# paTRICK-swk/D3DP

Hardware: AMD Instinct MI355X
Metric: pose-hypotheses/sec (H x clips) at F=243, J=17, H=20, K=10 (higher is better)
Workload: dtype f16x2-split operands on fp16 MFMA, f32 accumulate (fp32-class: meets 1e-3 mm)

## Files before the change

d3dp_amd/csrc/attention_x2.hip:

```cpp
#include "common.h"
#include "kernels.h"
#include "ta_common.h"
#include "attn_frag.h"

#ifndef D3DP_ATTN_OVERLAP
#define D3DP_ATTN_OVERLAP 0
#endif
#ifndef D3DP_ATTN_KPIPE
#define D3DP_ATTN_KPIPE 0
#endif
#ifndef D3DP_ATTN_MIXLO
#define D3DP_ATTN_MIXLO 0
#endif
#ifndef D3DP_ATTN_W16
#define D3DP_ATTN_W16 0
#endif
#ifndef D3DP_ATTN_STAMP
#define D3DP_ATTN_STAMP 0
#endif

namespace {

__device__ __forceinline__ f16x8 as_f16x8(bf16x8 v) { return __builtin_bit_cast(f16x8, v); }

// ... 732 lines not shown
          ph[e] = hh;
          pl[e] = (f16)fmaf(y, 1.0f, -(float)hh);
        }
        psum += __shfl_xor(psum, 16, 64);
        psum += __shfl_xor(psum, 32, 64);
        lrun = fmaf(lrun, alpha, psum);
#pragma unroll
        for (int dn = 0; dn < ND; ++dn) o[dn] *= alpha;
        if constexpr (HD == 64) {
          ta_tr_chunk<PLANE>(fv, t >> 1, ph, pl, o);
        } else {
          FragBasesT<HD> fc = fb;
#pragma unroll
          for (int dn = 0; dn < ND; ++dn) fc.v[dn] += (t >> 1) * 32 * H::ROWB;
          pv_chunk_x2_seq<0>(fc, PLANE, ph, pl, o);
        }
      }
    }
    if (active && q < n)
      store_o_x2<OUTS>(o, sc.onorm / lrun, out_v, (size_t)(tok0 + q * map.tok_stride), C, head * HD + fg * 4, sc.oplane);
  }
}

template <int OUTS, int HD = 64>
__global__ __launch_bounds__(256) void attn_spatial_x2_kernel(const float* __restrict__ qkv, void* __restrict__ out_v,
                                                              int n_prob, SeqMap map, int C, int heads, size_t plane_elems,
                                                              X2Scales sc) {
  using H = X2Head<HD>;
  constexpr int PLANE = 32 * H::ROWB, NQ = H::NQ, ND = HD / 16;
  __shared__ __attribute__((aligned(16))) char smem[4 * 2 * PLANE];
  const int n = map.n_tok;
  const int tid = threadIdx.x, lane = tid & 63, wave = tid >> 6;
  const int pid = blockIdx.x * 4 + wave;
  if (pid >= n_prob) return;
  const int seq = pid / heads, head = pid % heads;
  const int base = ta_seq_base(map, seq);
  const int ts = map.tok_stride;
  const size_t ldb = (size_t)12 * C;
  const char* rows = reinterpret_cast<const char*>(qkv) + (size_t)base * ldb;
  char* img = smem + wave * 2 * PLANE;
  const int fi = lane & 15, fg = lane >> 4;
  const int n_qt = (n + 15) >> 4;
  typename H::frag qh[2][NQ], ql[2][NQ], kh[2][NQ], kl[2][NQ];
#pragma unroll
  for (int t = 0; t < 2; ++t) {
    const char* row = rows + (size_t)min(t * 16 + fi, n - 1) * ts * ldb;
    load_q_x2<HD>(reinterpret_cast<const float*>(row) + head * HD, fg, qh[t], ql[t], sc.q);
    load_k_x2<HD>(reinterpret_cast<const f16*>(row + 4 * C) + head * HD, C, fg, kh[t], kl[t]);
  }
  for (int idx = lane; idx < (32 << H::LS); idx += 64) {
    const int row = idx >> H::LS, slot = idx & ((1 << H::LS) - 1);
    f16x8 vh = {}, vl = {};
    if (row < n) {
      const f16* src = reinterpret_cast<const f16*>(rows + (size_t)row * ts * ldb + 8 * C) + head * HD + slot * 8;
      vh = *reinterpret_cast<const f16x8*>(src);
      vl = *reinterpret_cast<const f16x8*>(src + C);
    }
    const int vo = row * H::ROWB + ((slot ^ v_slot_swizzle<HD>(row)) << 4);
    *reinterpret_cast<f16x8*>(img + vo) = vh;
    *reinterpret_cast<f16x8*>(img + PLANE + vo) = vl;
  }
  const FragBasesT<HD> fb = make_frag_bases<HD>(img, img, lane);
  const float inv_scale = sc.onorm;
  const float cexp = sc.cexp;
#pragma unroll
  for (int qt = 0; qt < 2; ++qt) {
    if (qt >= n_qt) break;
    const int q = qt * 16 + fi;
    f32x4 s[2];
#pragma unroll
    for (int t = 0; t < 2; ++t) {
      f32x4 a = {0.f, 0.f, 0.f, 0.f};
      if constexpr (HD == 64) {
        a = __builtin_amdgcn_mfma_f32_16x16x32_f16(kl[t][0], qh[qt][0], a, 0, 0, 0);
        a = __builtin_amdgcn_mfma_f32_16x16x32_f16(kl[t][1], qh[qt][1], a, 0, 0, 0);
        a = __builtin_amdgcn_mfma_f32_16x16x32_f16(kh[t][0], ql[qt][0], a, 0, 0, 0);
        a = __builtin_amdgcn_mfma_f32_16x16x32_f16(kh[t][1], ql[qt][1], a, 0, 0, 0);
        a = __builtin_amdgcn_mfma_f32_16x16x32_f16(kh[t][0], qh[qt][0], a, 0, 0, 0);
        a = __builtin_amdgcn_mfma_f32_16x16x32_f16(kh[t][1], qh[qt][1], a, 0, 0, 0);
      } else {
        a = x2_tile_scores(kh[t][0], kl[t][0], qh[qt][0], ql[qt][0]);
      }
      s[t] = a;
    }
    float mx = -INFINITY;
#pragma unroll
    for (int t = 0; t < 2; ++t)
#pragma unroll
      for (int r = 0; r < 4; ++r) {
        if (16 * t + 4 * fg + r >= n) s[t][r] = -INFINITY;
        mx = fmaxf(mx, s[t][r]);
      }
    mx = fmaxf(mx, __shfl_xor(mx, 16, 64));
    mx = fmaxf(mx, __shfl_xor(mx, 32, 64));
    const float nb = fmaf(-mx, cexp, 10.0f);
    float sum = 0.f;
    f16x8 ph[1], pl[1];
#pragma unroll
    for (int t = 0; t < 2; ++t)
#pragma unroll
      for (int r = 0; r < 4; ++r) {
        const float y = __builtin_amdgcn_exp2f(fmaf(s[t][r], cexp, nb));
        sum += y;
        const f16 h = (f16)y;
        ph[0][t * 4 + r] = h;
        pl[0][t * 4 + r] = (f16)fmaf(y, 1.0f, -(float)h);
      }
    sum += __shfl_xor(sum, 16, 64);
    sum += __shfl_xor(sum, 32, 64);
    f32x4 o[ND];
#pragma unroll
    for (int dn = 0; dn < ND; ++dn) o[dn] = (f32x4){0.f, 0.f, 0.f, 0.f};
    pv_chunk_x2_seq<0>(fb, PLANE, ph[0], pl[0], o);
    if (q < n) store_o_x2<OUTS>(o, inv_scale / sum, out_v, (size_t)(base + q * ts), C, head * HD + fg * 4, sc.oplane);
  }
}

__global__ void qkv_pack_x2_kernel(const float* __restrict__ src, char* __restrict__ dst, size_t T, int C, float sc) {
  const size_t total = T * (size_t)(3 * C / 4);
  for (size_t i = (size_t)blockIdx.x * blockDim.x + threadIdx.x; i < total; i += (size_t)gridDim.x * blockDim.x) {
    const size_t t = i / (3 * C / 4);
    const int c = (int)(i - t * (3 * C / 4)) * 4, region = c / C, cn = c - region * C;
    const float4 v = *reinterpret_cast<const float4*>(src + t * 3 * C + c);
    char* row = dst + t * 12 * C;
    if (region == 0) {
      *reinterpret_cast<float4*>(row + cn * 4) = v;
    } else {
      const float a[4] = {v.x, v.y, v.z, v.w};
      f16x4 ph, pl;
#pragma unroll
      for (int e = 0; e < 4; ++e) { f16 h, l; split2h_scaled(a[e] * sc, h, l); ph[e] = h; pl[e] = l; }
      *reinterpret_cast<f16x4*>(row + region * 4 * C + cn * 2) = ph;
      *reinterpret_cast<f16x4*>(row + region * 4 * C + 2 * C + cn * 2) = pl;
    }
  }
}

template <typename K>
// ... 19 lines not shown
    int per_cu = (int)((160 * 1024) / lds) < 2048 / (NW * 64) ? (int)((160 * 1024) / lds) : 2048 / (NW * 64);
    if constexpr (HD != 64) per_cu = x2_resident_per_cu(kern, NW * 64, per_cu);
    const int cus = d3dp_cu_count(dev);
    return cus < 0 ? cus : cus * per_cu;
  });
  if (n_wg < 0) return -3;
  const int n_prob = n_seq * heads;
#if D3DP_ATTN_W16
  if constexpr (NKT == 16 && HD == 64) {
    if (map.n_tok > 16 * (NKT - 1)) {
      hipLaunchKernelGGL((attn_temporal_x2_w16_kernel<OUTS>), dim3(n_prob < n_wg ? n_prob : n_wg), dim3(1024), 0, st,
                         (const float*)qkv, out, map, C, heads, plane, n_prob, sc);
      return 0;
    }
  }
#endif
  hipLaunchKernelGGL(kern, dim3(n_prob < n_wg ? n_prob : n_wg), dim3(NW * 64), 0, st, (const float*)qkv, out, map, C,
                     heads, plane, n_prob, sc);
  return 0;
}

template <int HD>
int launch_attn_x2_hd(int act, int axis, const void* qkv, void* out, int n_seq, SeqMap map, int C, int heads, float act_scale,
                      hipStream_t st) {
  const size_t plane = (size_t)n_seq * map.n_tok * C;
  const int n = map.n_tok;
  const X2Scales sc = {act_scale, (HD == 64 ? 0.125f : HD == 32 ? 0.17677669529663689f : 0.25f) * 1.44269504088896340736f / (act_scale * act_scale),
                       1.0f / act_scale, act_scale};
  if (axis == 0 && n <= 32) {
    const int n_prob = n_seq * heads;
    if (act == 3) hipLaunchKernelGGL((attn_spatial_x2_kernel<2, HD>), dim3((n_prob + 3) / 4), dim3(256), 0, st, (const float*)qkv, out, n_prob, map, C, heads, plane, sc);
    else hipLaunchKernelGGL((attn_spatial_x2_kernel<0, HD>), dim3((n_prob + 3) / 4), dim3(256), 0, st, (const float*)qkv, out, n_prob, map, C, heads, plane, sc);
    return 0;
  }
  if (n > 256) {
    const int groups = ((n + 15) / 16 + 7) / 8, n_work = n_seq * heads * groups;
    static PerDeviceOnce once[2];
    const int wgs = once[act == 3].get([&](int dev) {
      const int cus = d3dp_cu_count(dev);
      int per_cu = 2;
      if constexpr (HD != 64)
        per_cu = act == 3 ? x2_resident_per_cu(attn_temporal_x2_long_kernel<2, HD>, 512, 4) : x2_resident_per_cu(attn_temporal_x2_long_kernel<0, HD>, 512, 4);
      return cus < 0 ? cus : cus * per_cu;
    });
    if (wgs < 0) return -3;
    const dim3 grid(n_work < wgs ? n_work : wgs), blk(512);
    if (act == 3) hipLaunchKernelGGL((attn_temporal_x2_long_kernel<2, HD>), grid, blk, 0, st, (const float*)qkv, out, map, C, heads, groups, n_work, sc);
    else hipLaunchKernelGGL((attn_temporal_x2_long_kernel<0, HD>), grid, blk, 0, st, (const float*)qkv, out, map, C, heads, groups, n_work, sc);
    return 0;
  }
#define X2_CASE(NKT_)                                                                                         \
  return act == 3 ? launch_temporal_x2<NKT_, 2, HD>(qkv, out, n_seq, map, C, heads, plane, sc, st)            \
                  : launch_temporal_x2<NKT_, 0, HD>(qkv, out, n_seq, map, C, heads, plane, sc, st);
  if (n <= 32) { X2_CASE(2) }
  if (n <= 64) { X2_CASE(4) }
  if (n <= 128) { X2_CASE(8) }
  X2_CASE(16)
#undef X2_CASE
}

}

void d3dp_launch_qkv_pack_x2(const float* src, void* dst, size_t T, int C, float act_scale, hipStream_t st) {
  const size_t total = T * (size_t)(3 * C / 4);
  const unsigned blocks = (unsigned)((total + 255) / 256 < 8192 ? (total + 255) / 256 : 8192);
  hipLaunchKernelGGL(qkv_pack_x2_kernel, dim3(blocks ? blocks : 1), dim3(256), 0, st, src, (char*)dst, T, C, act_scale);
}

int d3dp_launch_attn_x2(int act, int axis, const void* qkv, void* out, int n_seq, SeqMap map, int C, int heads,
                        float act_scale, hipStream_t st) {
  if (heads < 1 || C % heads || map.n_tok < 1 || (act != 0 && act != 3) || !(act_scale > 0.f)) return -2;
  switch (C / heads) {
    case 64: return launch_attn_x2_hd<64>(act, axis, qkv, out, n_seq, map, C, heads, act_scale, st);
    case 32: return launch_attn_x2_hd<32>(act, axis, qkv, out, n_seq, map, C, heads, act_scale, st);
    case 16: return launch_attn_x2_hd<16>(act, axis, qkv, out, n_seq, map, C, heads, act_scale, st);
  }
  return -2;
}

#if D3DP_ATTN_STAMP
extern "C" __attribute__((visibility("default"))) int d3dp_debug_attn_stamps(unsigned long long* dst) {
  return (int)hipMemcpyFromSymbol(dst, HIP_SYMBOL(d3dp_attn_stamps), sizeof(unsigned long long) * 4 * 8 * 16 * 8);
}
#endif
```

d3dp_amd/csrc/capi.hip:

```cpp
#include <hip/hip_runtime.h>

#include <cmath>
#include <cstdarg>
#include <cstdio>
#include <cstdlib>
#include <cstring>
#include <string>
#include <vector>

#include "../../include/d3dp_hip.h"
#include "common.h"
#include "kernels.h"

namespace {

thread_local std::string g_err;

int fail(int code, const char* fmt, ...) {
  char buf[512];
  va_list ap;
  va_start(ap, fmt);
  vsnprintf(buf, sizeof buf, fmt, ap);
  va_end(ap);
  g_err = buf;
// ... 82 lines not shown
    const float w = fabsf(W[(size_t)n * K + k]);
    const double in = gamma ? sq * (double)fabsf(gamma[k]) + (double)fabsf(beta[k]) : c;
    const unsigned ib = f32_bits_up(in), wb = __float_as_uint(w);
    inmax = ib > inmax ? ib : inmax;
    wmax = wb > wmax ? wb : wmax;
    a += (double)w * in;
  }
#pragma unroll
  for (int o = 32; o > 0; o >>= 1) a += __shfl_xor(a, o, 64);
  inmax = wave_max_u(inmax);
  wmax = wave_max_u(wmax);
  if (lane == 0) {
    const unsigned sb = f32_bits_up((a + (double)fabsf(bias[n])) * (1.0 + 0x1p-40));
    atomicMax(o_sum, sb);
    if (o_tail && n >= n_tail) atomicMax(o_tail, sb);
    if (o_in) atomicMax(o_in, inmax);
    atomicMax(o_w, wmax);
  }
}
constexpr int kF16Slots = 11;

constexpr size_t kAlign = 256;
size_t align_up(size_t v) { return (v + kAlign - 1) / kAlign * kAlign; }

}

struct d3dp_ctx {
  d3dp_cfg cfg{};
  int device = 0;
  bool weights_set = false;
  float range_bound = 0.f;
  size_t ln_slice_floats = 0;
  unsigned* d_flag = nullptr;
  char* arena = nullptr;
  size_t arena_bytes = 0;
  const float *spos = nullptr, *tpos = nullptr, *ew = nullptr, *eb = nullptr, *freq = nullptr, *t1w = nullptr,
              *t1b = nullptr, *t3w = nullptr, *t3b = nullptr, *snw = nullptr, *snb = nullptr, *tnw = nullptr,
              *tnb = nullptr, *hnw = nullptr, *hnb = nullptr, *hw = nullptr, *hb = nullptr;
  std::vector<BlockDev> ste, tte;
  bool prof = false;
  struct Ev { hipEvent_t a, b; int cls; };
  std::vector<Ev> pool;
  size_t used = 0;
  int64_t counts[D3DP_PROFILE_CLASSES] = {0};
  double total_ms[D3DP_PROFILE_CLASSES] = {0};

  bool fast16() const { return cfg.mode == D3DP_MODE_FAST16; }
  bool fast() const { return cfg.mode == D3DP_MODE_FAST || fast16(); }
  int fast_f16 = 0;
  float fast_bound = 0.f;
  int exact_impl = 0;
  int exact_impl_req = 0;
  bool impl_fallback = false;
  bool train() const { return cfg.mode == D3DP_MODE_TRAIN; }
  bool exact() const { return !fast() && !train(); }
  bool x2() const { return exact() && exact_impl == 0; }
  bool long_rows = false;
  bool x2_attn() const {
    const int hd = cfg.channels / cfg.heads;
    return x2() && ((hd == 64 && (cfg.frames <= 256 || !long_rows)) || ((hd == 32 || hd == 16) && !long_rows));
  }
  bool fold_resid() const { return x2() && fold; }
  bool fold = true;
  bool fold_ln() const { return fold_resid() && fold_ln_on && 2 * cfg.hidden <= 2048; }
  bool fold_ln_on = false;
  bool defer_norm() const {
    return fold_resid() && defer && !fold_ln() && skew_d == 0 && pingpong == 0 && cfg.channels >= 96 && 3 * cfg.channels <= 2048;
  }
  bool defer = true;
  bool skew() const { return x2_attn() && skew_d > 0 && cfg.channels >= 128 * skew_d; }
  int skew_d = 0;
  int seq_pitch() const {
    const int fj = cfg.frames * cfg.joints;
    return (pad_override < 0 ? skew() : (pad_override > 0 && x2_attn())) ? (fj + 63) / 64 * 64 : fj;
  }
  int pad_override = -1;
  bool train_x2 = true;
  hipStream_t aux = nullptr;
  hipEvent_t ev_fork = nullptr, ev_done[2] = {nullptr, nullptr};
  bool train_overlap = true;
  int train_overlap_sets = 2;
  bool train_gelu_in_prep = true;
  bool train_ln_direct = true;
  bool train_wgrad_merged = true;
  bool train_tail_blocks = true;
  int train_attn_x2 = 2;
  int pingpong = 0;
  bool x3() const { return exact() && exact_impl == 1; }
  int act() const { return fast() ? (fast_f16 ? 4 : 1) : (x3() ? 2 : (x2() ? 3 : 0)); }
  size_t act_size() const { return fast() ? 2 : (x3() ? 6 : 4); }
  size_t wide_size() const { return fast() ? 2 : 4; }
  size_t y_size() const { return fast() ? 2 : 4; }
// ... 78 lines not shown
  Scope s(c, cls, st);
  if (c->fast()) return d3dp_launch_linear_bf16_stream(epi, out_f32, A, W, bias, out, M, N, K, st, c->fast_f16);
  if (c->x2()) {
    if (cls == P_QKV && c->x2_attn()) epi = EPI_QKV_PACK;
    const int skew_d = c->skew() && (epi == EPI_QKV_PACK || epi == EPI_GELU) ? c->skew_d : 0;
    const int rev = cls == P_PROJ ? X2_TILES_LAST_TO_FIRST : 0;
    return d3dp_launch_linear_f16x2(epi, A, W, bias, wu / a_scale, o_scale, (float*)out, out2 ? out2 : out, aux, c->d_flag, M, N,
                                    K, st, skew_d, c->pingpong | rev);
  }
  if (c->x3()) return d3dp_launch_linear_bf16x3(epi, A, W, bias, (float*)out, out, M, N, K, st);
  return d3dp_launch_linear_f32(epi, (const float*)A, (const float*)W, bias, (float*)out, M, N, K, st);
}

SeqMap spatial_map(int F, int J, int sp = 0) { return sp > F * J ? SeqMap{J, F, sp, J, 1} : SeqMap{J, 1, J, 0, 1}; }
SeqMap temporal_map(int F, int J, int sp = 0) { return SeqMap{F, J, sp > F * J ? sp : F * J, 1, J}; }

int attention(d3dp_ctx* c, int axis, const void* qkv, void* out, int n_bh, float s_kv, hipStream_t st) {
  const d3dp_cfg& g = c->cfg;
  Scope s(c, axis == 0 ? P_ATTN_S : P_ATTN_T, st);
  if (c->x2_attn())
    return d3dp_launch_attn_x2(3, axis, qkv, out, axis == 0 ? n_bh * g.frames : n_bh * g.joints,
                               axis == 0 ? spatial_map(g.frames, g.joints, c->seq_pitch())
                                         : temporal_map(g.frames, g.joints, c->seq_pitch()),
                               g.channels, g.heads, s_kv, st);
  const int hd = g.channels / g.heads;
  const bool fast_mfma = c->fast() && (hd == 64 || ((hd == 32 || hd == 16) && !c->long_rows));
  if (axis == 0) {
    if (fast_mfma && g.joints <= 32)
      return d3dp_launch_attn_spatial_bf16(qkv, out, n_bh * g.frames, spatial_map(g.frames, g.joints), g.channels,
                                           g.heads, st, c->fast_f16);
    if (fast_mfma && !c->long_rows)
      return d3dp_launch_attn_temporal_bf16(qkv, out, n_bh * g.frames, spatial_map(g.frames, g.joints), g.channels,
                                            g.heads, st, c->fast_f16);
    return d3dp_launch_attn_rows(c->act(), qkv, out, n_bh * g.frames, spatial_map(g.frames, g.joints), g.channels,
                                 g.heads, st);
  }
  if (fast_mfma && (g.frames <= 256 || !c->long_rows))
    return d3dp_launch_attn_temporal_bf16(qkv, out, n_bh * g.joints, temporal_map(g.frames, g.joints), g.channels,
                                          g.heads, st, c->fast_f16);
  if (c->exact() && g.channels / g.heads == 64 && g.frames <= 256)
    return d3dp_launch_attn_temporal_f32(c->act(), qkv, out, n_bh * g.joints, temporal_map(g.frames, g.joints),
                                         g.channels, g.heads, st);
  return d3dp_launch_attn_rows(c->act(), qkv, out, n_bh * g.joints, temporal_map(g.frames, g.joints), g.channels,
                               g.heads, st);
}

int run_block(d3dp_ctx* c, const BlockDev& w, int axis, float* x, void* y1, void* y, void* bufA, void* bufB, float* lnst,
              int n_bh, hipStream_t st, float* nstat = nullptr) {
  const d3dp_cfg& g = c->cfg;
  const int Tc = n_bh * c->seq_pitch(), C = g.channels;
  const float s_o = c->x2_attn() ? w.s_kv : kActScale;
  LAUNCH_TRY(linear(c, P_QKV, EPI_BIAS, 0, bufA, w.qkv_w, w.qkv_u, w.qkv_b, bufB, Tc, 3 * C, C, st, nullptr, nullptr, kActScale, s_o));
  LAUNCH_TRY(attention(c, axis, bufB, bufA, n_bh, s_o, st));
  const bool fold = c->fold_resid();
  if (c->fold_ln()) {
    float* slices = lnst;
    float* rowstat = lnst + (size_t)c->ln_slice_floats;
    LAUNCH_TRY(linear(c, P_PROJ, EPI_RESID_LN, 0, bufA, w.proj_w, w.proj_u, w.proj_b, x, Tc, C, C, st, y1, slices, s_o));
    {
      Scope s(c, P_LN, st);
      d3dp_launch_ln_combine(slices, rowstat, Tc, C, g.eps_block, st);
    }
    LAUNCH_TRY(linear(c, P_FC1, EPI_GELU_LN, 0, y1, w.fc1_w, w.fc1_u, w.fc1_c12, bufB, Tc, g.hidden, C, st, bufB, rowstat, kActScale, w.s_h));
  } else {
  if (nstat) LAUNCH_TRY(linear(c, P_PROJ, EPI_RESID_NORM, 0, bufA, w.proj_w, w.proj_u, w.proj_bgb, x, Tc, C, C, st, nullptr, nstat, s_o));
  else LAUNCH_TRY(linear(c, P_PROJ, fold ? EPI_RESID : EPI_BIAS, 0, bufA, w.proj_w, w.proj_u, w.proj_b, fold ? (void*)x : y1, Tc, C, C, st, nullptr, nullptr, s_o));
  {
    Scope s(c, P_LN, st);
    LAUNCH_TRY(d3dp_launch_ln(c->act(), x, fold ? nullptr : y1, 0, w.n2w, w.n2b, g.eps_block, bufA, Tc, C, st));
  }
  LAUNCH_TRY(linear(c, P_FC1, EPI_GELU, 0, bufA, w.fc1_w, w.fc1_u, w.fc1_b, bufB, Tc, g.hidden, C, st, nullptr, nullptr, kActScale, w.s_h));
  }
  LAUNCH_TRY(linear(c, P_FC2, fold ? EPI_RESID : EPI_BIAS, 0, bufB, w.fc2_w, w.fc2_u, w.fc2_b, fold ? (void*)x : y, Tc, C, g.hidden, st, nullptr, nullptr, w.s_h));
  return 0;
}

int read_switches(d3dp_ctx* c, bool width_inst) {
  const d3dp_cfg& g = c->cfg;
  const char* xf = getenv("D3DP_EXACT_IMPL");
  c->exact_impl = c->exact_impl_req = (xf && !strcmp(xf, "bf16x3")) ? 1 : (xf && !strcmp(xf, "f32")) ? 2 : 0;
  if (!width_inst) {
    if (c->exact_impl_req == 1)
      return fail(D3DP_ENOTSUP, "D3DP_EXACT_IMPL=bf16x3 exists for channels in {64,128,256,512}; channels=%d runs the fp32 implementation", g.channels);
    c->exact_impl = c->exact_impl_req = 2;
  }
  const char* lr = getenv("D3DP_LONG_ATTN");
  c->long_rows = lr && !strcmp(lr, "rows");
  const char* nf = getenv("D3DP_NO_FOLD");
  c->fold = !(nf && nf[0] == '1');
  const char* dn = getenv("D3DP_DEFER_NORM");
  c->defer = !(dn && dn[0] == '0');
  const char* ti = getenv("D3DP_TRAIN_IMPL");
  c->train_x2 = !(ti && !strcmp(ti, "f32")) && width_inst;
  const char* ov = getenv("D3DP_TRAIN_OVERLAP");
  c->train_overlap = !(ov && ov[0] == '0');
  c->train_overlap_sets = (ov && ov[0] == '1') ? 1 : 2;
  const char* tg = getenv("D3DP_TRAIN_GELU");
  c->train_gelu_in_prep = !(tg && !strcmp(tg, "pass"));
  const char* tw = getenv("D3DP_TRAIN_WGRAD");
  c->train_wgrad_merged = !(tw && !strcmp(tw, "each"));
  const char* tl = getenv("D3DP_TRAIN_LN_OPERAND");
  c->train_ln_direct = !(tl && !strcmp(tl, "pass"));
  const char* tt = getenv("D3DP_TRAIN_TAIL");
  c->train_tail_blocks = !(tt && !strcmp(tt, "split"));
  const char* ta = getenv("D3DP_TRAIN_ATTN");
  c->train_attn_x2 = (ta && !strcmp(ta, "f32")) ? 0 : (ta && !strcmp(ta, "x2t")) ? 1 : 2;
  if ((!c->train_gelu_in_prep || !c->train_wgrad_merged || !c->train_tail_blocks || !c->train_ln_direct) && !d3dp_x2_variants_built())
    return fail(D3DP_ENOTSUP, "D3DP_TRAIN_WGRAD=each / D3DP_TRAIN_TAIL=split / D3DP_TRAIN_GELU=pass / D3DP_TRAIN_LN_OPERAND=pass select superseded launch forms of the "
                              "training step that only the variants build honours (make -C d3dp_amd/csrc variants; "
                              "D3DP_LIB=d3dp_amd/lib/variants/libd3dp_variants.so)");
  {
    const char* sk = getenv("D3DP_X2_SKEW");
    const char* pp = getenv("D3DP_X2_PP");
    const char* wide = getenv("D3DP_X2_WIDE");
// ... 610 lines not shown
  if (!src || !dst) return fail(D3DP_EINVAL, "d3dp_op_split2: null argument");
  if (n % 32 != 0) return fail(D3DP_EINVAL, "d3dp_op_split2: n = %zu is not a multiple of 32 (the h2i layout is made of whole 32-column blocks)", n);
  d3dp_launch_split2(src, dst, n, scale, (hipStream_t)stream);
  HIP_TRY(hipGetLastError());
  return D3DP_OK;
}

int d3dp_op_attention(int32_t act_bf16, int32_t impl, int32_t axis, const void* qkv, void* out, int32_t n_bh, int32_t F,
                      int32_t J, int32_t C, int32_t heads, void* stream) {
  if (!qkv || !out || n_bh < 1) return fail(D3DP_EINVAL, "d3dp_op_attention: bad argument");
  hipStream_t st = (hipStream_t)stream;
  if (act_bf16 != 0 && act_bf16 != 1 && act_bf16 != 4) return fail(D3DP_EINVAL, "act_bf16 must be 0, 1 or 4 (fp16)");
  const int f16 = act_bf16 == 4;
  if (impl == 2) {
    if (act_bf16) return fail(D3DP_EINVAL, "split-fp16 attention takes fp32 activations");
    if (heads < 1 || C % heads || (C / heads != 64 && C / heads != 32 && C / heads != 16))
      return fail(D3DP_ENOTSUP, "impl 2 (split-fp16 attention) takes head dims 64, 32 and 16; C=%d heads=%d is head dim %d (the row "
                                "kernel, impl 0, takes it)", C, heads, heads > 0 ? C / heads : 0);
    void* packed = nullptr;
    const size_t T = (size_t)n_bh * F * J;
    HIP_TRY(hipMallocAsync(&packed, T * 12 * (size_t)C, st));
    d3dp_launch_qkv_pack_x2((const float*)qkv, packed, T, C, kActScale, st);
    const int rc = d3dp_launch_attn_x2(0, axis, packed, out, axis == 0 ? n_bh * F : n_bh * J,
                                       axis == 0 ? spatial_map(F, J) : temporal_map(F, J), C, heads, kActScale, st);
    HIP_TRY(hipFreeAsync(packed, st));
    LAUNCH_TRY(rc);
  } else if (impl == 1 && act_bf16 && (heads < 1 || C % heads || (C / heads != 64 && C / heads != 32 && C / heads != 16))) {
    return fail(D3DP_ENOTSUP, "impl 1 on 2-byte rows takes head dims 64, 32 and 16; C=%d heads=%d is head dim %d (the row kernel, "
                              "impl 0, takes it)", C, heads, heads > 0 ? C / heads : 0);
  } else if (axis == 0 && impl == 1) {
    if (!act_bf16) return fail(D3DP_EINVAL, "MFMA spatial attention needs bf16 activations");
    if (J <= 32) LAUNCH_TRY(d3dp_launch_attn_spatial_bf16(qkv, out, n_bh * F, spatial_map(F, J), C, heads, st, f16));
    else if (J > 256) return fail(D3DP_ENOTSUP, "MFMA spatial attention takes up to 256 joints; J=%d", J);
    else LAUNCH_TRY(d3dp_launch_attn_temporal_bf16(qkv, out, n_bh * F, spatial_map(F, J), C, heads, st, f16));
  } else if (axis == 0) LAUNCH_TRY(d3dp_launch_attn_rows(act_bf16, qkv, out, n_bh * F, spatial_map(F, J), C, heads, st));
  else if (impl == 1 && !act_bf16) {
    LAUNCH_TRY(d3dp_launch_attn_temporal_f32(0, qkv, out, n_bh * J, temporal_map(F, J), C, heads, st));
  } else if (impl == 1) {
    if (!act_bf16) return fail(D3DP_EINVAL, "MFMA temporal attention needs bf16 activations");
    LAUNCH_TRY(d3dp_launch_attn_temporal_bf16(qkv, out, n_bh * J, temporal_map(F, J), C, heads, st, f16));
  } else LAUNCH_TRY(d3dp_launch_attn_rows(act_bf16, qkv, out, n_bh * J, temporal_map(F, J), C, heads, st));
  HIP_TRY(hipGetLastError());
  return D3DP_OK;
}

int d3dp_op_layernorm(int32_t out_bf16, const float* x, const float* w, const float* b, float eps, void* out, int32_t T,
                      int32_t C, void* stream) {
// ... 756 lines not shown
```

d3dp_amd/csrc/kernels.h:

```cpp
#pragma once
#include <hip/hip_runtime.h>
#include <stdint.h>

#include <mutex>

struct PerDeviceOnce {
  static constexpr int kMaxDev = 64;
  std::mutex mu;
  int val[kMaxDev] = {0};
  template <class F> int get(F&& fn) {
    int dev = 0;
    if (hipGetDevice(&dev) != hipSuccess || dev < 0 || dev >= kMaxDev) return -3;
    std::lock_guard<std::mutex> lock(mu);
    if (val[dev] <= 0) {
      const int v = fn(dev);
      if (v <= 0) return v < 0 ? v : -3;
      val[dev] = v;
    }
    return val[dev];
  }
};
inline int d3dp_cu_count(int dev) {
  hipDeviceProp_t prop;
  if (hipGetDeviceProperties(&prop, dev) != hipSuccess || prop.multiProcessorCount < 1) return -3;
// ... 60 lines not shown
void d3dp_launch_sum_partials_many(const D3dpSumTable& tb, hipStream_t st);
constexpr int D3DP_WPREP_MAX = 64;
struct D3dpWPrepItem { const float* w; int N, K, slot, pad; size_t off; };
struct D3dpWPrepTable { D3dpWPrepItem it[D3DP_WPREP_MAX]; int n; };
int d3dp_launch_wprep(const D3dpWPrepTable& tb, void* rows_base, void* cols_base, unsigned* amax, float* unscale, hipStream_t st);
void d3dp_launch_sum_partials(const float* part, float* out, size_t n, int Z, hipStream_t st);
void d3dp_launch_sum_partials_bias(const float* part, const float* bias, float* out, size_t n, int N, int Z, hipStream_t st,
                                   unsigned* amax = nullptr, int amax_pos = 0);
int d3dp_launch_linear_f32_splitk(const float* A, const float* W, float* out, int M, int N, int K, hipStream_t st, float* part,
                                  size_t part_floats);
int d3dp_launch_linear_f32(int epi, const float* A, const float* W, const float* bias, float* out, int M, int N,
                           int K, hipStream_t st);

struct SeqMap { int n_tok, inner, outer_stride, inner_stride, tok_stride; };
int d3dp_launch_attn_rows(int act_bf16, const void* qkv, void* out, int n_seq, SeqMap map, int C, int heads,
                          hipStream_t st, unsigned* amax = nullptr);
int d3dp_launch_attn_temporal_f32(int act, const void* qkv, void* out, int n_seq, SeqMap map, int C, int heads,
                                  hipStream_t st);
int d3dp_launch_attn_temporal_bf16(const void* qkv, void* out, int n_seq, SeqMap map, int C, int heads,
                                   hipStream_t st, int f16 = 0);
int d3dp_launch_attn_spatial_bf16(const void* qkv, void* out, int n_seq, SeqMap map, int C, int heads, hipStream_t st,
                                  int f16 = 0);
int d3dp_launch_attn_x2(int act, int axis, const void* qkv, void* out, int n_seq, SeqMap map, int C, int heads,
                        float act_scale, hipStream_t st);
void d3dp_launch_qkv_pack_x2(const float* src, void* dst, size_t T, int C, float act_scale, hipStream_t st);

int d3dp_launch_time_mlp(const int64_t* t, const float* freq, const float* w1, const float* b1, const float* w2,
                         const float* b2, float* temb, int B, int C, hipStream_t st);
int d3dp_launch_embed_ln(int act_bf16, const float* x2d, const float* x3d, const float* temb, const float* ew,
                         const float* eb, const float* spos, const float* lnw, const float* lnb, float eps, float* x,
                         void* xn, int seq0, int n_seq, int H, int F, int J, int C, hipStream_t st, int SP = 0);
int d3dp_launch_ln(int act_bf16, float* x, const void* yadd, int write_x, const float* w, const float* b, float eps,
                   void* xn, int T, int C, hipStream_t st);
int d3dp_launch_ln2(int act_bf16, float* x, const void* yadd0, const void* yadd, const float* wa, const float* ba, const float* pos,
                    const float* wb, const float* bb, float eps, void* xn, int T, int C, int F, int J, hipStream_t st,
                    int SP = 0);
int d3dp_launch_ln2_defer(int act_bf16, const float* x, const float* wa, const float* ba, const float* wb, const float* bb, float eps,
                          void* xn, float* stat, int T, int C, hipStream_t st);
int d3dp_launch_head(int act_bf16, const float* x, const void* yadd0, const void* yadd, const float* wa, const float* ba, float eps_a, const float* wh,
                     const float* bh, float eps_h, const float* w, const float* b, float* out, int T, int C,
                     hipStream_t st, int FJ = 0, int SP = 0);

int d3dp_launch_ddim_pre(const float* img, float* xt2, const int* perm, float scale, int B, int per_b, int J,
                         hipStream_t st);
int d3dp_launch_ddim_post(const float* pred2, const float* img, const float* noise, const int* perm, float scale,
                          double sqrt_recip, double sqrt_recipm1, float c_xstart, float c_noise, float sigma,
                          int last, float* x_start, size_t xs_bstride, float* img_next, int B, int per_b, int J,
                          hipStream_t st);
int d3dp_launch_q_sample(const float* x0, const float* noise, const double* a, const double* b, float scale,
                         float* out, int B, int per_b, hipStream_t st);

int d3dp_launch_jpma(const float* pred, const float* traj, const float* cam, const float* gt2d, const float* gt3d,
                     float* agg, int* sel, float* err_sel, float* err_min, float* win, float* jbest, float* mean,
                     int h_offset, int B, int K, int H, int F, int J, int root_joint, int linear, hipStream_t st,
                     int h_inner = 0, size_t outer_stride = 0);

// ... 66 lines not shown
```

d3dp_amd/csrc/pointwise.hip:

```cpp
#include <type_traits>

#include "common.h"
#include "kernels.h"

namespace {

#ifndef NT_STREAMS
#define NT_STREAMS 1
#endif
#ifndef NT_Y
#define NT_Y 1
#endif

template <int C> struct Row {
  static constexpr int NV = C / 64;
  static constexpr bool V4 = (NV % 4 == 0);
  static __device__ __forceinline__ int elem(int lane, int i) {
    if constexpr (V4) return ((i >> 2) * 64 + lane) * 4 + (i & 3);
    else return i * 64 + lane;
  }
  static __device__ __forceinline__ void load(const float* p, int lane, float* v) {
    if constexpr (V4) {
#pragma unroll
      for (int g = 0; g < NV / 4; ++g) {
// ... 233 lines not shown
template <int C, typename XN>
__global__ __launch_bounds__(256) void ln2_defer_kernel(const float* __restrict__ x, const float* __restrict__ wa,
                                                        const float* __restrict__ ba, const float* __restrict__ wb,
                                                        const float* __restrict__ bb, float eps,
                                                        typename ActOut<C, XN>::ptr xn, float2* __restrict__ stat,
                                                        size_t plane, int T) {
  using R = Row<C>;
  const int lane = threadIdx.x & 63;
  const int wave = __builtin_amdgcn_readfirstlane(threadIdx.x >> 6);
  float wav[R::NV], bav[R::NV], wbv[R::NV], bbv[R::NV];
  R::load(wa, lane, wav);
  R::load(ba, lane, bav);
  R::load(wb, lane, wbv);
  R::load(bb, lane, bbv);
  for (int it = 0; it < kDeferRows; ++it) {
    const int tok = (blockIdx.x * kDeferRows + it) * 4 + wave;
    if (tok >= T) break;
    float v[R::NV], y[R::NV], z[R::NV];
    if (NT_STREAMS) R::load_nt(x + (size_t)tok * C, lane, v); else R::load(x + (size_t)tok * C, lane, v);
    const float2 st = R::norm_r(v, wav, bav, eps, y);
    if (lane == 0) stat[tok] = st;
    R::norm_r(y, wbv, bbv, eps, z);
    ActOut<C, XN>::st(xn, plane, (size_t)tok * C, lane, z);
  }
}

constexpr int kRowTokens = 8;

template <int C, typename XN>
__global__ __launch_bounds__(256) void embed_ln_kernel(const float* __restrict__ x2d, const float* __restrict__ x3d,
                                                       const float* __restrict__ temb, const float* __restrict__ ew,
                                                       const float* __restrict__ eb, const float* __restrict__ spos,
                                                       const float* __restrict__ lnw, const float* __restrict__ lnb,
                                                       float eps, float* __restrict__ x,
                                                       typename ActOut<C, XN>::ptr xn, size_t plane, int seq0,
                                                       int n_seq, int H, int F, int J, int SP) {
  using R = Row<C>;
  const int lane = threadIdx.x & 63;
  const int wave = __builtin_amdgcn_readfirstlane(threadIdx.x >> 6);
  const int FJ = F * J, T = n_seq * SP;
  float w5[R::NV][5], ebv[R::NV], lw[R::NV], lb[R::NV];
#pragma unroll
  for (int i = 0; i < R::NV; ++i) {
    const float* wr = ew + R::elem(lane, i) * 5;
#pragma unroll
    for (int k = 0; k < 5; ++k) w5[i][k] = wr[k];
// ... 297 lines not shown
                         const float* eb, const float* spos, const float* lnw, const float* lnb, float eps, float* x,
                         void* xn, int seq0, int n_seq, int H, int F, int J, int C, hipStream_t st, int SP) {
  if (SP <= 0) SP = F * J;
  if (SP < F * J) return -1;
  const int T = n_seq * SP;
  dim3 g((T + 3) / 4), blk(256);
  const size_t plane = (size_t)T * C;
  if (!width_instantiated(C)) {
    if (act_bf16 != 0) return -2;
    DISPATCH_G(C, hipLaunchKernelGGL((embed_ln_g_kernel<NVM>), g, blk, 0, st, x2d, x3d, temb, ew, eb, spos, lnw, lnb, eps, x, (float*)xn, seq0, n_seq, H, F, J, SP, C))
    return 0;
  }
  const dim3 gk((T + 4 * kRowTokens - 1) / (4 * kRowTokens));
  DISPATCH_C(C,
    if (act_bf16 == 1) hipLaunchKernelGGL((embed_ln_kernel<CC, bf16>), gk, blk, 0, st, x2d, x3d, temb, ew, eb, spos, lnw, lnb, eps, x, (bf16*)xn, plane, seq0, n_seq, H, F, J, SP);
    else if (act_bf16 == 4) hipLaunchKernelGGL((embed_ln_kernel<CC, f16>), gk, blk, 0, st, x2d, x3d, temb, ew, eb, spos, lnw, lnb, eps, x, (f16*)xn, plane, seq0, n_seq, H, F, J, SP);
    else if (act_bf16 == 2) hipLaunchKernelGGL((embed_ln_kernel<CC, b3>), gk, blk, 0, st, x2d, x3d, temb, ew, eb, spos, lnw, lnb, eps, x, (bf16*)xn, plane, seq0, n_seq, H, F, J, SP);
    else if (act_bf16 == 3) hipLaunchKernelGGL((embed_ln_kernel<CC, h2>), gk, blk, 0, st, x2d, x3d, temb, ew, eb, spos, lnw, lnb, eps, x, (f16*)xn, plane, seq0, n_seq, H, F, J, SP);
    else hipLaunchKernelGGL((embed_ln_kernel<CC, float>), gk, blk, 0, st, x2d, x3d, temb, ew, eb, spos, lnw, lnb, eps, x, (float*)xn, plane, seq0, n_seq, H, F, J, SP))
  return 0;
}

int d3dp_launch_ln(int act_bf16, float* x, const void* yadd, int write_x, const float* w, const float* b, float eps,
                   void* xn, int T, int C, hipStream_t st) {
  dim3 g((T + 3) / 4), blk(256);
  const size_t plane = (size_t)T * C;
  if (!width_instantiated(C)) {
    if (act_bf16 != 0) return -2;
    DISPATCH_G(C, hipLaunchKernelGGL((ln_g_kernel<NVM>), g, blk, 0, st, x, (const float*)yadd, w, b, eps, (float*)xn, T, C, write_x))
    return 0;
  }
  DISPATCH_C(C,
    if (act_bf16 == 1) hipLaunchKernelGGL((ln_kernel<CC, bf16, bf16>), g, blk, 0, st, x, (const bf16*)yadd, w, b, eps, (bf16*)xn, plane, T, write_x);
    else if (act_bf16 == 4) hipLaunchKernelGGL((ln_kernel<CC, f16, f16>), g, blk, 0, st, x, (const f16*)yadd, w, b, eps, (f16*)xn, plane, T, write_x);
    else if (act_bf16 == 2) hipLaunchKernelGGL((ln_kernel<CC, b3, float>), g, blk, 0, st, x, (const float*)yadd, w, b, eps, (bf16*)xn, plane, T, write_x);
    else if (act_bf16 == 3) hipLaunchKernelGGL((ln_kernel<CC, h2, float>), g, blk, 0, st, x, (const float*)yadd, w, b, eps, (f16*)xn, plane, T, write_x);
    else hipLaunchKernelGGL((ln_kernel<CC, float, float>), g, blk, 0, st, x, (const float*)yadd, w, b, eps, (float*)xn, plane, T, write_x))
  return 0;
}

int d3dp_launch_ln2(int act_bf16, float* x, const void* yadd0, const void* yadd, const float* wa, const float* ba, const float* pos,
                    const float* wb, const float* bb, float eps, void* xn, int T, int C, int F, int J, hipStream_t st, int SP) {
  if (SP <= 0) SP = F * J;
  dim3 g((T + 3) / 4), blk(256);
  const size_t plane = (size_t)T * C;
  if (!width_instantiated(C)) {
    if (act_bf16 != 0) return -2;
    DISPATCH_G(C, hipLaunchKernelGGL((ln2_g_kernel<NVM>), g, blk, 0, st, x, (const float*)yadd0, (const float*)yadd, wa, ba, pos, wb, bb, eps, (float*)xn, T, C, F, J, SP))
    return 0;
// ... 37 lines not shown
```

Measured before the change: 50.69.

## Add register-lean spatial attention path with occupancy bound and multi-row LN kernel

Spatial x2 attention becomes a shared body with a TILEWISE variant that keeps only one Q tile in registers. It prefetches Q and V into registers before the LDS writes and splits the second Q tile during the first tile's PV, and sets a min-waves launch bound per head dim to raise occupancy. A new LN kernel processes several rows per wave with hoisted weight loads for the no-residual h2 case. Both are on by default behind D3DP_WAVE_OCC; the risk is register spills under the tighter launch bound and less overlap of Q loads.

```diff
diff --git a/d3dp_amd/csrc/attention_x2.hip b/d3dp_amd/csrc/attention_x2.hip
--- a/d3dp_amd/csrc/attention_x2.hip
+++ b/d3dp_amd/csrc/attention_x2.hip
@@ -778,15 +778,14 @@
   }
 }
 
-template <int OUTS, int HD = 64>
-__global__ __launch_bounds__(256) void attn_spatial_x2_kernel(const float* __restrict__ qkv, void* __restrict__ out_v,
-                                                              int n_prob, SeqMap map, int C, int heads, size_t plane_elems,
-                                                              X2Scales sc) {
+template <int OUTS, int HD, bool TILEWISE>
+__device__ __forceinline__ void attn_spatial_x2_body(char* smem, const float* __restrict__ qkv, void* __restrict__ out_v,
+                                                     int n_prob, const SeqMap& map, int C, int heads, const X2Scales& sc) {
   using H = X2Head<HD>;
   constexpr int PLANE = 32 * H::ROWB, NQ = H::NQ, ND = HD / 16;
-  __shared__ __attribute__((aligned(16))) char smem[4 * 2 * PLANE];
   const int n = map.n_tok;
-  const int tid = threadIdx.x, lane = tid & 63, wave = tid >> 6;
+  const int tid = threadIdx.x, lane = tid & 63;
+  const int wave = TILEWISE ? __builtin_amdgcn_readfirstlane(tid >> 6) : tid >> 6;
   const int pid = blockIdx.x * 4 + wave;
   if (pid >= n_prob) return;
   const int seq = pid / heads, head = pid % heads;
@@ -797,24 +796,74 @@
   char* img = smem + wave * 2 * PLANE;
   const int fi = lane & 15, fg = lane >> 4;
   const int n_qt = (n + 15) >> 4;
-  typename H::frag qh[2][NQ], ql[2][NQ], kh[2][NQ], kl[2][NQ];
-#pragma unroll
-  for (int t = 0; t < 2; ++t) {
-    const char* row = rows + (size_t)min(t * 16 + fi, n - 1) * ts * ldb;
-    load_q_x2<HD>(reinterpret_cast<const float*>(row) + head * HD, fg, qh[t], ql[t], sc.q);
-    load_k_x2<HD>(reinterpret_cast<const f16*>(row + 4 * C) + head * HD, C, fg, kh[t], kl[t]);
-  }
-  for (int idx = lane; idx < (32 << H::LS); idx += 64) {
-    const int row = idx >> H::LS, slot = idx & ((1 << H::LS) - 1);
-    f16x8 vh = {}, vl = {};
-    if (row < n) {
-      const f16* src = reinterpret_cast<const f16*>(rows + (size_t)row * ts * ldb + 8 * C) + head * HD + slot * 8;
-      vh = *reinterpret_cast<const f16x8*>(src);
-      vl = *reinterpret_cast<const f16x8*>(src + C);
-    }
-    const int vo = row * H::ROWB + ((slot ^ v_slot_swizzle<HD>(row)) << 4);
-    *reinterpret_cast<f16x8*>(img + vo) = vh;
-    *reinterpret_cast<f16x8*>(img + PLANE + vo) = vl;
+  constexpr int QT = TILEWISE ? 1 : 2;
+  typename H::frag qh[QT][NQ], ql[QT][NQ], kh[2][NQ], kl[2][NQ];
+  [[maybe_unused]] f32x4 qr[H::NQL];
+  [[maybe_unused]] auto q_request = [&](int t) {
+    const float* p = reinterpret_cast<const float*>(rows + (size_t)min(t * 16 + fi, n - 1) * ts * ldb) + head * HD + fg * (HD == 16 ? 4 : 8);
+#pragma unroll
+    for (int i = 0; i < H::NQL; ++i) qr[i] = *reinterpret_cast<const f32x4*>(p + (i >> 1) * 32 + (i & 1) * 4);
+  };
+  [[maybe_unused]] auto q_split = [&]() {
+    if constexpr (HD == 16) {
+      x2_split4(qr[0], qh[0][0], ql[0][0], sc.q);
+    } else {
+#pragma unroll
+      for (int half = 0; half < NQ; ++half)
+        ta_split8(make_float4(qr[2 * half][0], qr[2 * half][1], qr[2 * half][2], qr[2 * half][3]),
+                  make_float4(qr[2 * half + 1][0], qr[2 * half + 1][1], qr[2 * half + 1][2], qr[2 * half + 1][3]), qh[0][half],
+                  ql[0][half], sc.q);
+    }
+  };
+  if constexpr (!TILEWISE) {
+#pragma unroll
+    for (int t = 0; t < 2; ++t) {
+      const char* row = rows + (size_t)min(t * 16 + fi, n - 1) * ts * ldb;
+      load_q_x2<HD>(reinterpret_cast<const float*>(row) + head * HD, fg, qh[t], ql[t], sc.q);
+      load_k_x2<HD>(reinterpret_cast<const f16*>(row + 4 * C) + head * HD, C, fg, kh[t], kl[t]);
+    }
+    for (int idx = lane; idx < (32 << H::LS); idx += 64) {
+      const int row = idx >> H::LS, slot = idx & ((1 << H::LS) - 1);
+      f16x8 vh = {}, vl = {};
+      if (row < n) {
+        const f16* src = reinterpret_cast<const f16*>(rows + (size_t)row * ts * ldb + 8 * C) + head * HD + slot * 8;
+        vh = *reinterpret_cast<const f16x8*>(src);
+        vl = *reinterpret_cast<const f16x8*>(src + C);
+      }
+      const int vo = row * H::ROWB + ((slot ^ v_slot_swizzle<HD>(row)) << 4);
+      *reinterpret_cast<f16x8*>(img + vo) = vh;
+      *reinterpret_cast<f16x8*>(img + PLANE + vo) = vl;
+    }
+  } else {
+    constexpr int NV = (32 << H::LS) / 64, RPS = 64 >> H::LS;
+    q_request(0);
+#pragma unroll
+    for (int t = 0; t < 2; ++t) {
+      if (t >= n_qt) break;
+      load_k_x2<HD>(reinterpret_cast<const f16*>(rows + (size_t)min(t * 16 + fi, n - 1) * ts * ldb + 4 * C) + head * HD, C, fg, kh[t], kl[t]);
+    }
+    f16x8 vh[NV], vl[NV];
+    const int vrow = lane >> H::LS, slot = lane & ((1 << H::LS) - 1);
+#pragma unroll
+    for (int j = 0; j < NV; ++j) {
+      vh[j] = f16x8{}; vl[j] = f16x8{};
+      if (j * RPS < n) {
+        const f16* src = reinterpret_cast<const f16*>(rows + (size_t)min(vrow + j * RPS, n - 1) * ts * ldb + 8 * C) + head * HD + slot * 8;
+        vh[j] = *reinterpret_cast<const f16x8*>(src);
+        vl[j] = *reinterpret_cast<const f16x8*>(src + C);
+      }
+    }
+    __builtin_amdgcn_sched_barrier(0);
+#pragma unroll
+    for (int j = 0; j < NV; ++j) {
+      const int row = vrow + j * RPS;
+      const int vo = row * H::ROWB + ((slot ^ v_slot_swizzle<HD>(row)) << 4);
+      *reinterpret_cast<f16x8*>(img + vo) = row < n ? vh[j] : f16x8{};
+      *reinterpret_cast<f16x8*>(img + PLANE + vo) = row < n ? vl[j] : f16x8{};
+    }
+    q_split();
+    if (n_qt > 1) q_request(1);
+    __builtin_amdgcn_sched_barrier(0);
   }
   const FragBasesT<HD> fb = make_frag_bases<HD>(img, img, lane);
   const float inv_scale = sc.onorm;
@@ -823,19 +872,22 @@
   for (int qt = 0; qt < 2; ++qt) {
     if (qt >= n_qt) break;
     const int q = qt * 16 + fi;
+    constexpr int QI = TILEWISE ? 0 : 1;
     f32x4 s[2];
 #pragma unroll
     for (int t = 0; t < 2; ++t) {
       f32x4 a = {0.f, 0.f, 0.f, 0.f};
-      if constexpr (HD == 64) {
-        a = __builtin_amdgcn_mfma_f32_16x16x32_f16(kl[t][0], qh[qt][0], a, 0, 0, 0);
-        a = __builtin_amdgcn_mfma_f32_16x16x32_f16(kl[t][1], qh[qt][1], a, 0, 0, 0);
-        a = __builtin_amdgcn_mfma_f32_16x16x32_f16(kh[t][0], ql[qt][0], a, 0, 0, 0);
-        a = __builtin_amdgcn_mfma_f32_16x16x32_f16(kh[t][1], ql[qt][1], a, 0, 0, 0);
-        a = __builtin_amdgcn_mfma_f32_16x16x32_f16(kh[t][0], qh[qt][0], a, 0, 0, 0);
-        a = __builtin_amdgcn_mfma_f32_16x16x32_f16(kh[t][1], qh[qt][1], a, 0, 0, 0);
+      if (TILEWISE && t >= n_qt) {
+        a = (f32x4){-INFINITY, -INFINITY, -INFINITY, -INFINITY};
+      } else if constexpr (HD == 64) {
+        a = __builtin_amdgcn_mfma_f32_16x16x32_f16(kl[t][0], qh[qt * QI][0], a, 0, 0, 0);
+        a = __builtin_amdgcn_mfma_f32_16x16x32_f16(kl[t][1], qh[qt * QI][1], a, 0, 0, 0);
+        a = __builtin_amdgcn_mfma_f32_16x16x32_f16(kh[t][0], ql[qt * QI][0], a, 0, 0, 0);
+        a = __builtin_amdgcn_mfma_f32_16x16x32_f16(kh[t][1], ql[qt * QI][1], a, 0, 0, 0);
+        a = __builtin_amdgcn_mfma_f32_16x16x32_f16(kh[t][0], qh[qt * QI][0], a, 0, 0, 0);
+        a = __builtin_amdgcn_mfma_f32_16x16x32_f16(kh[t][1], qh[qt * QI][1], a, 0, 0, 0);
       } else {
-        a = x2_tile_scores(kh[t][0], kl[t][0], qh[qt][0], ql[qt][0]);
+        a = x2_tile_scores(kh[t][0], kl[t][0], qh[qt * QI][0], ql[qt * QI][0]);
       }
       s[t] = a;
     }
@@ -867,9 +919,27 @@
     f32x4 o[ND];
 #pragma unroll
     for (int dn = 0; dn < ND; ++dn) o[dn] = (f32x4){0.f, 0.f, 0.f, 0.f};
+    if constexpr (TILEWISE) {
+      if (qt == 0 && n_qt > 1) q_split();
+    }
     pv_chunk_x2_seq<0>(fb, PLANE, ph[0], pl[0], o);
     if (q < n) store_o_x2<OUTS>(o, inv_scale / sum, out_v, (size_t)(base + q * ts), C, head * HD + fg * 4, sc.oplane);
   }
+}
+template <int HD> constexpr int kSpatialWaves = HD == 64 ? 5 : HD == 32 ? 6 : 8;
+template <int OUTS, int HD = 64>
+__global__ __launch_bounds__(256, kSpatialWaves<HD>) void attn_spatial_x2_kernel(const float* __restrict__ qkv, void* __restrict__ out_v,
+                                                                                 int n_prob, SeqMap map, int C, int heads,
+                                                                                 size_t plane_elems, X2Scales sc) {
+  __shared__ __attribute__((aligned(16))) char smem[4 * 2 * 32 * X2Head<HD>::ROWB];
+  attn_spatial_x2_body<OUTS, HD, true>(smem, qkv, out_v, n_prob, map, C, heads, sc);
+}
+template <int OUTS, int HD = 64>
+__global__ __launch_bounds__(256) void attn_spatial_x2_wide_kernel(const float* __restrict__ qkv, void* __restrict__ out_v,
+                                                                   int n_prob, SeqMap map, int C, int heads, size_t plane_elems,
+                                                                   X2Scales sc) {
+  __shared__ __attribute__((aligned(16))) char smem[4 * 2 * 32 * X2Head<HD>::ROWB];
+  attn_spatial_x2_body<OUTS, HD, false>(smem, qkv, out_v, n_prob, map, C, heads, sc);
 }
 
 __global__ void qkv_pack_x2_kernel(const float* __restrict__ src, char* __restrict__ dst, size_t T, int C, float sc) {
@@ -935,15 +1005,21 @@
 
 template <int HD>
 int launch_attn_x2_hd(int act, int axis, const void* qkv, void* out, int n_seq, SeqMap map, int C, int heads, float act_scale,
-                      hipStream_t st) {
+                      hipStream_t st, int spatial_wide) {
   const size_t plane = (size_t)n_seq * map.n_tok * C;
   const int n = map.n_tok;
   const X2Scales sc = {act_scale, (HD == 64 ? 0.125f : HD == 32 ? 0.17677669529663689f : 0.25f) * 1.44269504088896340736f / (act_scale * act_scale),
                        1.0f / act_scale, act_scale};
   if (axis == 0 && n <= 32) {
     const int n_prob = n_seq * heads;
-    if (act == 3) hipLaunchKernelGGL((attn_spatial_x2_kernel<2, HD>), dim3((n_prob + 3) / 4), dim3(256), 0, st, (const float*)qkv, out, n_prob, map, C, heads, plane, sc);
-    else hipLaunchKernelGGL((attn_spatial_x2_kernel<0, HD>), dim3((n_prob + 3) / 4), dim3(256), 0, st, (const float*)qkv, out, n_prob, map, C, heads, plane, sc);
+    const dim3 grid((n_prob + 3) / 4), blk(256);
+    if (spatial_wide) {
+      if (act == 3) hipLaunchKernelGGL((attn_spatial_x2_wide_kernel<2, HD>), grid, blk, 0, st, (const float*)qkv, out, n_prob, map, C, heads, plane, sc);
+      else hipLaunchKernelGGL((attn_spatial_x2_wide_kernel<0, HD>), grid, blk, 0, st, (const float*)qkv, out, n_prob, map, C, heads, plane, sc);
+      return 0;
+    }
+    if (act == 3) hipLaunchKernelGGL((attn_spatial_x2_kernel<2, HD>), grid, blk, 0, st, (const float*)qkv, out, n_prob, map, C, heads, plane, sc);
+    else hipLaunchKernelGGL((attn_spatial_x2_kernel<0, HD>), grid, blk, 0, st, (const float*)qkv, out, n_prob, map, C, heads, plane, sc);
     return 0;
   }
   if (n > 256) {
@@ -981,12 +1057,12 @@
 }
 
 int d3dp_launch_attn_x2(int act, int axis, const void* qkv, void* out, int n_seq, SeqMap map, int C, int heads,
-                        float act_scale, hipStream_t st) {
+                        float act_scale, hipStream_t st, int spatial_wide) {
   if (heads < 1 || C % heads || map.n_tok < 1 || (act != 0 && act != 3) || !(act_scale > 0.f)) return -2;
   switch (C / heads) {
-    case 64: return launch_attn_x2_hd<64>(act, axis, qkv, out, n_seq, map, C, heads, act_scale, st);
-    case 32: return launch_attn_x2_hd<32>(act, axis, qkv, out, n_seq, map, C, heads, act_scale, st);
-    case 16: return launch_attn_x2_hd<16>(act, axis, qkv, out, n_seq, map, C, heads, act_scale, st);
+    case 64: return launch_attn_x2_hd<64>(act, axis, qkv, out, n_seq, map, C, heads, act_scale, st, spatial_wide);
+    case 32: return launch_attn_x2_hd<32>(act, axis, qkv, out, n_seq, map, C, heads, act_scale, st, spatial_wide);
+    case 16: return launch_attn_x2_hd<16>(act, axis, qkv, out, n_seq, map, C, heads, act_scale, st, spatial_wide);
   }
   return -2;
 }
diff --git a/d3dp_amd/csrc/capi.hip b/d3dp_amd/csrc/capi.hip
--- a/d3dp_amd/csrc/capi.hip
+++ b/d3dp_amd/csrc/capi.hip
@@ -128,6 +128,11 @@
 
 constexpr size_t kAlign = 256;
 size_t align_up(size_t v) { return (v + kAlign - 1) / kAlign * kAlign; }
+
+bool wave_occ_switch() {
+  const char* wo = getenv("D3DP_WAVE_OCC");
+  return !(wo && wo[0] == '0');
+}
 
 }
 
@@ -174,6 +179,7 @@
     return fold_resid() && defer && !fold_ln() && skew_d == 0 && pingpong == 0 && cfg.channels >= 96 && 3 * cfg.channels <= 2048;
   }
   bool defer = true;
+  bool wave_occ = true;
   bool skew() const { return x2_attn() && skew_d > 0 && cfg.channels >= 128 * skew_d; }
   int skew_d = 0;
   int seq_pitch() const {
@@ -298,7 +304,7 @@
     return d3dp_launch_attn_x2(3, axis, qkv, out, axis == 0 ? n_bh * g.frames : n_bh * g.joints,
                                axis == 0 ? spatial_map(g.frames, g.joints, c->seq_pitch())
                                          : temporal_map(g.frames, g.joints, c->seq_pitch()),
-                               g.channels, g.heads, s_kv, st);
+                               g.channels, g.heads, s_kv, st, !c->wave_occ);
   const int hd = g.channels / g.heads;
   const bool fast_mfma = c->fast() && (hd == 64 || ((hd == 32 || hd == 16) && !c->long_rows));
   if (axis == 0) {
@@ -343,7 +349,7 @@
   else LAUNCH_TRY(linear(c, P_PROJ, fold ? EPI_RESID : EPI_BIAS, 0, bufA, w.proj_w, w.proj_u, w.proj_b, fold ? (void*)x : y1, Tc, C, C, st, nullptr, nullptr, s_o));
   {
     Scope s(c, P_LN, st);
-    LAUNCH_TRY(d3dp_launch_ln(c->act(), x, fold ? nullptr : y1, 0, w.n2w, w.n2b, g.eps_block, bufA, Tc, C, st));
+    LAUNCH_TRY(d3dp_launch_ln(c->act(), x, fold ? nullptr : y1, 0, w.n2w, w.n2b, g.eps_block, bufA, Tc, C, st, c->wave_occ));
   }
   LAUNCH_TRY(linear(c, P_FC1, EPI_GELU, 0, bufA, w.fc1_w, w.fc1_u, w.fc1_b, bufB, Tc, g.hidden, C, st, nullptr, nullptr, kActScale, w.s_h));
   }
@@ -366,6 +372,7 @@
   c->fold = !(nf && nf[0] == '1');
   const char* dn = getenv("D3DP_DEFER_NORM");
   c->defer = !(dn && dn[0] == '0');
+  c->wave_occ = wave_occ_switch();
   const char* ti = getenv("D3DP_TRAIN_IMPL");
   c->train_x2 = !(ti && !strcmp(ti, "f32")) && width_inst;
   const char* ov = getenv("D3DP_TRAIN_OVERLAP");
@@ -1022,7 +1029,8 @@
     HIP_TRY(hipMallocAsync(&packed, T * 12 * (size_t)C, st));
     d3dp_launch_qkv_pack_x2((const float*)qkv, packed, T, C, kActScale, st);
     const int rc = d3dp_launch_attn_x2(0, axis, packed, out, axis == 0 ? n_bh * F : n_bh * J,
-                                       axis == 0 ? spatial_map(F, J) : temporal_map(F, J), C, heads, kActScale, st);
+                                       axis == 0 ? spatial_map(F, J) : temporal_map(F, J), C, heads, kActScale, st,
+                                       !wave_occ_switch());
     HIP_TRY(hipFreeAsync(packed, st));
     LAUNCH_TRY(rc);
   } else if (impl == 1 && act_bf16 && (heads < 1 || C % heads || (C / heads != 64 && C / heads != 32 && C / heads != 16))) {
diff --git a/d3dp_amd/csrc/kernels.h b/d3dp_amd/csrc/kernels.h
--- a/d3dp_amd/csrc/kernels.h
+++ b/d3dp_amd/csrc/kernels.h
@@ -106,7 +106,7 @@
 int d3dp_launch_attn_spatial_bf16(const void* qkv, void* out, int n_seq, SeqMap map, int C, int heads, hipStream_t st,
                                   int f16 = 0);
 int d3dp_launch_attn_x2(int act, int axis, const void* qkv, void* out, int n_seq, SeqMap map, int C, int heads,
-                        float act_scale, hipStream_t st);
+                        float act_scale, hipStream_t st, int spatial_wide = 0);
 void d3dp_launch_qkv_pack_x2(const float* src, void* dst, size_t T, int C, float act_scale, hipStream_t st);
 
 int d3dp_launch_time_mlp(const int64_t* t, const float* freq, const float* w1, const float* b1, const float* w2,
@@ -115,7 +115,7 @@
                          const float* eb, const float* spos, const float* lnw, const float* lnb, float eps, float* x,
                          void* xn, int seq0, int n_seq, int H, int F, int J, int C, hipStream_t st, int SP = 0);
 int d3dp_launch_ln(int act_bf16, float* x, const void* yadd, int write_x, const float* w, const float* b, float eps,
-                   void* xn, int T, int C, hipStream_t st);
+                   void* xn, int T, int C, hipStream_t st, int wave_rows = 0);
 int d3dp_launch_ln2(int act_bf16, float* x, const void* yadd0, const void* yadd, const float* wa, const float* ba, const float* pos,
                     const float* wb, const float* bb, float eps, void* xn, int T, int C, int F, int J, hipStream_t st,
                     int SP = 0);
diff --git a/d3dp_amd/csrc/pointwise.hip b/d3dp_amd/csrc/pointwise.hip
--- a/d3dp_amd/csrc/pointwise.hip
+++ b/d3dp_amd/csrc/pointwise.hip
@@ -279,6 +279,26 @@
     if (lane == 0) stat[tok] = st;
     R::norm_r(y, wbv, bbv, eps, z);
     ActOut<C, XN>::st(xn, plane, (size_t)tok * C, lane, z);
+  }
+}
+
+template <int C>
+__global__ __launch_bounds__(256) void ln_rows_kernel(const float* __restrict__ x, const float* __restrict__ w,
+                                                      const float* __restrict__ b, float eps, f16* __restrict__ xn, size_t plane,
+                                                      int T) {
+  using R = Row<C>;
+  const int lane = threadIdx.x & 63;
+  const int wave = __builtin_amdgcn_readfirstlane(threadIdx.x >> 6);
+  float wv[R::NV], bv[R::NV];
+  R::load(w, lane, wv);
+  R::load(b, lane, bv);
+  for (int it = 0; it < kDeferRows; ++it) {
+    const int tok = (blockIdx.x * kDeferRows + it) * 4 + wave;
+    if (tok >= T) break;
+    float v[R::NV], y[R::NV];
+    if (NT_STREAMS) R::load_nt(x + (size_t)tok * C, lane, v); else R::load(x + (size_t)tok * C, lane, v);
+    R::norm_r(v, wv, bv, eps, y);
+    ActOut<C, h2>::st(xn, plane, (size_t)tok * C, lane, y);
   }
 }
 
@@ -622,9 +642,14 @@
 }
 
 int d3dp_launch_ln(int act_bf16, float* x, const void* yadd, int write_x, const float* w, const float* b, float eps,
-                   void* xn, int T, int C, hipStream_t st) {
+                   void* xn, int T, int C, hipStream_t st, int wave_rows) {
   dim3 g((T + 3) / 4), blk(256);
   const size_t plane = (size_t)T * C;
+  if (wave_rows && act_bf16 == 3 && !yadd && width_instantiated(C)) {
+    const dim3 gr((T + 4 * kDeferRows - 1) / (4 * kDeferRows));
+    DISPATCH_C(C, hipLaunchKernelGGL((ln_rows_kernel<CC>), gr, blk, 0, st, x, w, b, eps, (f16*)xn, plane, T))
+    return 0;
+  }
   if (!width_instantiated(C)) {
     if (act_bf16 != 0) return -2;
     DISPATCH_G(C, hipLaunchKernelGGL((ln_g_kernel<NVM>), g, blk, 0, st, x, (const float*)yadd, w, b, eps, (float*)xn, T, C, write_x))
```

Result: no change. 50.67 (-0.0%).
